# MarioPasc/MU-Diff

Measured on AMD Instinct MI355X. Metric: 256x256 slices/sec (4-step dual-gen reverse), higher is better.
Workload: dtype f32 (convs/attention: fp16 hi+lo split MFMA x3; 3x3 convs that fill the chip: fp16 hi.hi + e4m3 cross terms; fp32 accumulate); 1 GPU; BASELINE config 3 (BraTS-shaped test-split batches of 32; model and slice shapes of config 2): 4-step dual-generator sampling, 256x256, nf=64, ch_mult 1-2-4, 32 slices per GPU per step, batch-sharded over 1 GPU(s), weights replicated; batch=32, hipgraph=True

## Files before the change

### include/mudiff_hip.h

```cpp
#ifndef MUDIFF_HIP_H
#define MUDIFF_HIP_H

#include <stdint.h>

#ifdef __cplusplus
extern "C" {
#endif

#define MUD_OK 0
#define MUD_ERR_ARG 1
#define MUD_ERR_LAUNCH 2
#define MUD_ERR_UNSUPPORTED 3

#define MUD_ACT_NONE 0
#define MUD_ACT_SIGMOID 1
#define MUD_ACT_TANH 2
#define MUD_ACT_SILU 3
#define MUD_ACT_LRELU 4

#define MUD_PRO_NONE 0
#define MUD_PRO_AFFINE 1
#define MUD_PRO_AFFINE_SILU 2
#define MUD_PRO_LRELU 3
#define MUD_PRO_UP2_AFFINE_SILU 4
// ... 56 lines not shown
  int sub2;
  double* stats; int stats_ld;
  int emul_cout;
  const double* gn_sums; int gn_sums_ld;
  int gn_G; float gn_eps; double gn_count;
  const float* gn_gamma; const float* gn_beta;
  int64_t gn_bstride;
  void* splitk_ws; int64_t splitk_ws_bytes;
  unsigned* splitk_counters; int splitk_ncounters;
  const void* skip_w; const float* skip_bias; float* skip_out; int skip_ldo;
  int prec; int w_exp;
  int res_up2; float res_k[4];
  int in_up2; float in_k[4];
  int in_s2d;
} mud_conv_args;

int mud_conv2d_direct(const mud_conv_args* a, void* stream);

int64_t mud_packed_weight_bytes(int ks, int Cin, int Cout);
int mud_pack_weights(const float* src, int64_t s_tap, int64_t s_ci, int64_t s_co, int64_t src_bstride,
                     int ks, int Cin, int Cout, int nbatch, void* dst, void* stream);
int mud_pack_weights_prec(const float* src, int64_t s_tap, int64_t s_ci, int64_t s_co, int64_t src_bstride,
                          int ks, int Cin, int Cout, int nbatch, int prec, int w_exp, void* dst, void* stream);
int64_t mud_packed_weight_bytes_prec(int ks, int Cin, int Cout, int prec);
int mud_conv2d_mfma(const mud_conv_args* a, void* stream);
int mud_conv2d_mfma_prec_supported(const mud_conv_args* a, int prec);
int64_t mud_conv2d_mfma_splitk_bytes(const mud_conv_args* a);
int mud_conv2d_mfma_res_up2_supported(const mud_conv_args* a);
int mud_conv2d_mfma_in_up2_supported(const mud_conv_args* a);
int mud_conv2d_mfma_in_s2d_supported(const mud_conv_args* a);

typedef struct mud_census_args {
  const float* x; int B, H, W, C, ldx;
  const float* pro_scale; const float* pro_shift; int pro_ld; int pro_mode;
} mud_census_args;
typedef struct mud_census_out {
  uint64_t n, n_over, n_under, n_fp16_over, amax_bits;
} mud_census_out;
int mud_e4m3_census(const mud_census_args* a, mud_census_out* out, void* stream);

int mud_upfirdn2d(const float* in, int64_t planes, int H, int W, const float* kernel, int kh, int kw,
                  int up_x, int up_y, int down_x, int down_y, int pad_x0, int pad_x1, int pad_y0, int pad_y1,
                  float* out, void* stream);
int mud_fir_nhwc(const float* x, int B, int H, int W, int C, int ldx, const float* kernel_host, int kh, int kw,
                 int up, int down, int pad0, int pad1,
                 const float* pro_scale, const float* pro_shift, int pro_ld, int pro_mode,
                 float* out_h, int ldh, float* out_x, int ldxo, void* stream);

int mud_minibatch_stddev(const float* x, int B, int64_t hw, int C, int ld, int group, float* out, void* stream);

int mud_attention_supported(int C);
int64_t mud_attention_ws_bytes(int B, int N, int C);
int mud_attention(const float* qkv, int B, int N, int C, int ld, float scale, float* out, int ldo, void* ws, void* stream);

int mud_softmax_rows(float* s, int64_t rows, int n, int ld, void* stream);
int mud_mul(const float* a, int lda, const float* b, int ldb, float* out, int ldo, int64_t npix, int C, void* stream);
int mud_gate_mix(const float* g, int ldg, const float* att, int lda, const float* other, int ldb,
                 float* out, int ldo, int B, int64_t hw, int C, double* stats, int stats_ld, void* stream);

int mud_fourier_embedding(const float* t, const float* W, float* out, int B, int n, void* stream);
int mud_resize_bilinear(const float* in, int64_t planes, int H, int W, int Ho, int Wo, float* out, void* stream);
int mud_affine_clamp(const float* x, int64_t n, float scale, float shift, float lo, float hi, float* out, void* stream);

int64_t mud_value_range_ws_bytes(void);
int mud_value_range(const float* a, int64_t na, const float* b, int64_t nb, float* out, void* ws, void* stream);
int mud_quantize_u8(const float* x, int64_t n, float lo, float range, uint8_t* out, void* stream);
int64_t mud_slice_metrics_ws_bytes(int n, int H, int W);
int mud_slice_metrics_u8(const uint8_t* pred, const uint8_t* gt, int n, int H, int W, int64_t* sse, int64_t* sae, double* ssim_sum,
                         void* ws, int64_t ws_bytes, void* stream);

#define MUD_VM_MAX_REGIONS 8
#define MUD_VM_NQ 8
#define MUD_VM_N 0
#define MUD_VM_SSE 1
#define MUD_VM_SAE 2
#define MUD_VM_N_INT 3
#define MUD_VM_SSIM 4
#define MUD_VM_SS 5
#define MUD_VM_SS2 6
#define MUD_VM_SSE_STD 7
int64_t mud_volume_metrics_ws_bytes(int Z, int X, int Y, int nreg);
int mud_volume_metrics(const float* pred, const float* gt, const uint8_t* region, const float* std, int Z, int X, int Y, int nreg,
                       double* sums, void* ws, int64_t ws_bytes, void* stream);

int64_t mud_lpips_packed_bytes(void);
int mud_lpips_pack(const float* table, void* const* conv_w, void* const* conv_b, void* const* lin_w, void* packed, void* stream);
int64_t mud_lpips_ws_bytes(int n, int H, int W);
int mud_lpips_u8(const uint8_t* pred, const uint8_t* gt, int n, int H, int W, const void* packed, double* out, void* ws,
                 int64_t ws_bytes, void* stream);

int mud_randn_keyed(float* out, int rows, int64_t row_len, const int64_t* keys, uint64_t seed, int step, int kind, void* stream);
int mud_ensemble_stats(const float* samples, int n, int N, int64_t hw, float scale, float shift, float lo, float hi, float* mean,
                       float* std, void* stream);

#define MUD_ENSEMBLE_MAX_QUANTILES 8
#define MUD_ENSEMBLE_QUANTILES_MAX_N 64
int mud_ensemble_quantiles(const float* samples, int n, int N, int64_t hw, float scale, float shift, float lo, float hi, const double* q,
                           int K, float* out, void* stream);

#define MUD_VC_NC 5
#define MUD_VC_NS 2
#define MUD_VC_PARTS 16
#define MUD_VC_N 0
#define MUD_VC_BELOW 1
#define MUD_VC_ABOVE 2
#define MUD_VC_INSIDE 3
// ... 136 lines not shown
```

### mu-diff_amd/csrc/attention.hip

```cpp
#include "mud_common.h"
#include <stdlib.h>

template <int C16>
struct AtGeo {
  static constexpr int C = 16 * C16;
  static constexpr int CT = (C16 + 1) / 2;
  static constexpr int CP = CT * 32;
  static constexpr int KROW = C * 4 + 16;
  static constexpr int VROW = 144;
  static constexpr int KT = 32 * KROW, VT = CP * VROW;
  static constexpr int BUF = KT + VT;
  static constexpr int LDS_BYTES = 2 * BUF;
  static constexpr int KITEMS = 32 * (C / 4), KN = (KITEMS + 255) / 256;
  static constexpr int VITEMS = CP * 8, VN = (VITEMS + 255) / 256;
};

template <int C16>
__global__ __launch_bounds__(256, 1) void k_attention(const float* __restrict__ qkv, int N, int ld, float scale_log2,
                                                       float* __restrict__ out, int ldo, int tiles_per_split, float* __restrict__ part) {
  using G = AtGeo<C16>;
  constexpr int C = G::C, CT = G::CT;
  extern __shared__ __attribute__((aligned(16))) char smem[];
  const int tid = threadIdx.x, lane = tid & 63, wave = tid >> 6, r = lane & 31, hh = lane >> 5;
  const int b = blockIdx.y;
// ... 170 lines not shown
    }

    if (more) stash_v(nxt);
    __syncthreads();
  }

  const float l_tot = l_run + __shfl_xor(l_run, 32, 64);
  if (part) {
    if (qi < N) {
      float* pp = part + (((int64_t)b * gridDim.z + blockIdx.z) * N + qi) * (C + 4);
#pragma unroll
      for (int ct = 0; ct < CT; ++ct)
#pragma unroll
        for (int q4 = 0; q4 < 4; ++q4) {
          const int c0 = ct * 32 + 8 * q4 + 4 * hh;
          if (c0 < C) *(f32x4*)(pp + c0) = f32x4{o[ct][4 * q4], o[ct][4 * q4 + 1], o[ct][4 * q4 + 2], o[ct][4 * q4 + 3]};
        }
      if (hh == 0) { pp[C] = m_run; pp[C + 1] = l_tot; }
    }
    return;
  }
  const float inv = 1.0f / l_tot;
  if (qi < N) {
    float* op = out + ((int64_t)b * N + qi) * ldo;
#pragma unroll
    for (int ct = 0; ct < CT; ++ct)
#pragma unroll
      for (int q4 = 0; q4 < 4; ++q4) {
        const int c0 = ct * 32 + 8 * q4 + 4 * hh;
        if (c0 < C) {
          f32x4 v = {o[ct][4 * q4] * inv, o[ct][4 * q4 + 1] * inv, o[ct][4 * q4 + 2] * inv, o[ct][4 * q4 + 3] * inv};
          *(f32x4*)(op + c0) = v;
        }
      }
  }
}

template <int C16>
struct At2Geo {
  static_assert(C16 % 4 == 0 && C16 >= 8, "pair variant: C in {128, 256}");
  static constexpr int C = 16 * C16;
  static constexpr int H16 = C16 / 2;
  static constexpr int CTH = C16 / 4;
  static constexpr int KROW = C * 4 + 16;
  static constexpr int VROW = 144;
  static constexpr int KT = 32 * KROW, VT = C * VROW;
  static constexpr int V_OFF = 2 * KT, X_OFF = V_OFF + VT;
  static constexpr int LDS_BYTES = X_OFF + 8 * 4096;
  static constexpr int KN = (32 * (C / 4)) / 512;
  static constexpr int VN = (C * 8) / 512;
  static_assert(KN * 512 == 32 * (C / 4) && VN * 512 == C * 8, "staging split");
};

template <int C16>
__global__ __launch_bounds__(512, 2) void k_attention_pair(const float* __restrict__ qkv, int N, int ld, float scale_log2,
                                                            float* __restrict__ out, int ldo, int tiles_per_split, float* __restrict__ part) {
  using G = At2Geo<C16>;
  constexpr int C = G::C, H16 = G::H16, CTH = G::CTH;
  extern __shared__ __attribute__((aligned(16))) char smem[];
  const int tid = threadIdx.x, lane = tid & 63, wave = tid >> 6, r = lane & 31, hh = lane >> 5;
  const int pair = wave & 3, half = wave >> 2;
  const int b = blockIdx.y;
  const int qi = blockIdx.x * 128 + pair * 32 + r;
  const float* base = qkv + (int64_t)b * N * ld;
  const int kt0 = blockIdx.z * tiles_per_split;
  const int ntiles = min((N + 31) / 32, kt0 + tiles_per_split);

  mud_h16x8 qh[H16], ql[H16];
#pragma unroll
  for (int s = 0; s < H16; ++s) {
    f32x4 v0 = {0.f, 0.f, 0.f, 0.f}, v1 = {0.f, 0.f, 0.f, 0.f};
    if (qi < N) {
      const float* qp = base + (int64_t)qi * ld + 16 * (half * H16 + s) + 8 * hh;
      v0 = *(const f32x4*)qp;
      v1 = *(const f32x4*)(qp + 4);
    }
#pragma unroll
    for (int e = 0; e < 4; ++e) {
      mud_h16 h0, h1, l0, l1;
      mud_split1(v0[e], h0, l0);
      mud_split1(v1[e], h1, l1);
      qh[s][e] = h0; qh[s][4 + e] = h1;
      ql[s][e] = l0; ql[s][4 + e] = l1;
    }
  }

  const __amdgpu_buffer_rsrc_t rsrc = __builtin_amdgcn_make_buffer_rsrc((void*)base, 0, (int)((int64_t)N * ld * 4 < 0x7fffffffLL ? (int64_t)N * ld * 4 : 0x7fffffffLL), 0x00020000);
  constexpr int KJ = 512 / (C / 4);
  constexpr int VG = 512 / C;
  const unsigned kvoff = (unsigned)(((tid / (C / 4)) * ld + C + 4 * (tid % (C / 4))) * 4);
  const unsigned vvoff = (unsigned)((2 * C + (tid % C)) * 4 + (4 * (tid / C)) * ld * 4);
  f32x4 kraw[G::KN];
  float vraw[G::VN][4];
  auto fetch_k = [&](int kt) {
#pragma unroll
    for (int i = 0; i < G::KN; ++i)
      kraw[i] = __builtin_bit_cast(f32x4, __builtin_amdgcn_raw_buffer_load_b128(rsrc, kvoff, (kt * 32 + KJ * i) * ld * 4, 0));
  };
  auto fetch_v = [&](int kt) {
#pragma unroll
    for (int i = 0; i < G::VN; ++i)
#pragma unroll
      for (int u = 0; u < 4; ++u)
        vraw[i][u] = __builtin_bit_cast(float, __builtin_amdgcn_raw_buffer_load_b32(rsrc, vvoff, (kt * 32 + 4 * VG * i + u) * ld * 4, 0));
  };
  auto stash_k = [&](char* buf) {
#pragma unroll
    for (int i = 0; i < G::KN; ++i) {
      const int item = tid + 512 * i, j = item / (C / 4), c4 = item % (C / 4);
      mud_h16x4 hi, lo;
      mud_split4(kraw[i], hi, lo);
      *(mud_h16x4*)(buf + j * G::KROW + c4 * 8) = hi;
      *(mud_h16x4*)(buf + j * G::KROW + C * 2 + c4 * 8) = lo;
    }
  };
  auto stash_v = [&]() {
#pragma unroll
    for (int i = 0; i < G::VN; ++i) {
      const int item = tid + 512 * i, c = item % C, g = item / C;
      const int jj = (4 * g) & 15, s = (4 * g) >> 4, h = (jj >> 2) & 1, blk = (jj >> 3) & 1;
      mud_h16x4 hi, lo;
#pragma unroll
      for (int u = 0; u < 4; ++u) {
        mud_h16 th, tl;
        mud_split1(vraw[i][u], th, tl);
        hi[u] = th;
        lo[u] = tl;
      }
      char* p = smem + G::V_OFF + c * G::VROW + s * 32 + h * 16 + blk * 8;
      *(mud_h16x4*)p = hi;
      *(mud_h16x4*)(p + 64) = lo;
    }
  };

  f32x16 o[CTH];
#pragma unroll
  for (int ct = 0; ct < CTH; ++ct)
#pragma unroll
    for (int i = 0; i < 16; ++i) o[ct][i] = 0.f;
  float m_run = -INFINITY, l_run = 0.f;
  f32x4* const xmine = (f32x4*)(smem + G::X_OFF + wave * 4096) + lane;
  const f32x4* const xpeer = (const f32x4*)(smem + G::X_OFF + (wave ^ 4) * 4096) + lane;

  fetch_k(kt0);
  stash_k(smem);
  fetch_v(kt0);
  stash_v();
  __syncthreads();

  for (int kt = kt0; kt < ntiles; ++kt) {
    const char* cur = smem + ((kt - kt0) & 1) * G::KT;
    char* nxt = smem + ((kt - kt0 + 1) & 1) * G::KT;
    const bool more = kt + 1 < ntiles;
    if (more) fetch_k(kt + 1);

    f32x16 st;
#pragma unroll
    for (int i = 0; i < 16; ++i) st[i] = 0.f;
#pragma unroll
    for (int s = 0; s < H16; ++s) {
      const char* kp = cur + r * G::KROW + (16 * (half * H16 + s) + 8 * hh) * 2;
      const mud_h16x8 kh = *(const mud_h16x8*)kp;
      const mud_h16x8 kl = *(const mud_h16x8*)(kp + C * 2);
      st = mud_mfma16(kl, qh[s], st);
      st = mud_mfma16(kh, ql[s], st);
      st = mud_mfma16(kh, qh[s], st);
    }
#pragma unroll
    for (int q4 = 0; q4 < 4; ++q4) xmine[q4 * 64] = f32x4{st[4 * q4], st[4 * q4 + 1], st[4 * q4 + 2], st[4 * q4 + 3]};
    if (more) {
      stash_k(nxt);
      fetch_v(kt + 1);
    }
    __syncthreads();
#pragma unroll
    for (int q4 = 0; q4 < 4; ++q4) {
      const f32x4 p = xpeer[q4 * 64];
      if (half == 0) { st[4 * q4] += p[0]; st[4 * q4 + 1] += p[1]; st[4 * q4 + 2] += p[2]; st[4 * q4 + 3] += p[3]; }
      else { st[4 * q4] = p[0] + st[4 * q4]; st[4 * q4 + 1] = p[1] + st[4 * q4 + 1]; st[4 * q4 + 2] = p[2] + st[4 * q4 + 2]; st[4 * q4 + 3] = p[3] + st[4 * q4 + 3]; }
    }

    float mt = -INFINITY;
#pragma unroll
    for (int i = 0; i < 16; ++i) {
      const int key = kt * 32 + (i & 3) + 8 * (i >> 2) + 4 * hh;
      st[i] = key < N ? st[i] * scale_log2 : -INFINITY;
      mt = fmaxf(mt, st[i]);
    }
    mt = fmaxf(mt, __shfl_xor(mt, 32, 64));
    const float m_new = fmaxf(m_run, mt);
    const float alpha = __builtin_amdgcn_exp2f(m_run - m_new);
    float psum = 0.f;
#pragma unroll
    for (int i = 0; i < 16; ++i) {
      st[i] = __builtin_amdgcn_exp2f(st[i] - m_new);
      psum += st[i];
    }
    l_run = l_run * alpha + psum;
    m_run = m_new;
    if (!__all(alpha == 1.0f)) {
#pragma unroll
      for (int ct = 0; ct < CTH; ++ct)
#pragma unroll
        for (int i = 0; i < 16; ++i) o[ct][i] *= alpha;
    }
    mud_h16x8 ph[2], pl[2];
#pragma unroll
    for (int s2 = 0; s2 < 2; ++s2)
#pragma unroll
      for (int e = 0; e < 8; ++e) {
        const float p = st[8 * s2 + e];
        const mud_h16 t = (mud_h16)p;
        ph[s2][e] = t;
        pl[s2][e] = (mud_h16)(p - (float)t);
      }

#pragma unroll
    for (int ct = 0; ct < CTH; ++ct) {
#pragma unroll
      for (int s2 = 0; s2 < 2; ++s2) {
        const char* vp = smem + G::V_OFF + ((half * CTH + ct) * 32 + r) * G::VROW + s2 * 32 + hh * 16;
        const mud_h16x8 vh = *(const mud_h16x8*)vp;
        const mud_h16x8 vl = *(const mud_h16x8*)(vp + 64);
        o[ct] = mud_mfma16(vl, ph[s2], o[ct]);
        o[ct] = mud_mfma16(vh, pl[s2], o[ct]);
        o[ct] = mud_mfma16(vh, ph[s2], o[ct]);
      }
    }
    __syncthreads();
    if (more) stash_v();
  }

  const float l_tot = l_run + __shfl_xor(l_run, 32, 64);
  if (part) {
    if (qi < N) {
      float* pp = part + (((int64_t)b * gridDim.z + blockIdx.z) * N + qi) * (C + 4);
#pragma unroll
      for (int ct = 0; ct < CTH; ++ct)
#pragma unroll
        for (int q4 = 0; q4 < 4; ++q4) {
          const int c0 = (half * CTH + ct) * 32 + 8 * q4 + 4 * hh;
          *(f32x4*)(pp + c0) = f32x4{o[ct][4 * q4], o[ct][4 * q4 + 1], o[ct][4 * q4 + 2], o[ct][4 * q4 + 3]};
        }
      if (hh == 0 && half == 0) { pp[C] = m_run; pp[C + 1] = l_tot; }
    }
    return;
  }
  const float inv = 1.0f / l_tot;
  if (qi < N) {
    float* op = out + ((int64_t)b * N + qi) * ldo;
#pragma unroll
    for (int ct = 0; ct < CTH; ++ct)
#pragma unroll
      for (int q4 = 0; q4 < 4; ++q4) {
        const int c0 = (half * CTH + ct) * 32 + 8 * q4 + 4 * hh;
        *(f32x4*)(op + c0) = f32x4{o[ct][4 * q4] * inv, o[ct][4 * q4 + 1] * inv, o[ct][4 * q4 + 2] * inv, o[ct][4 * q4 + 3] * inv};
      }
  }
}

__global__ __launch_bounds__(256) void k_attention_combine(const float* __restrict__ part, int N, int C, int nsplit, float* __restrict__ out, int ldo) {
  const int C4 = C / 4;
  const unsigned t = blockIdx.x * 256u + threadIdx.x;
  if (t >= (unsigned)(N * C4)) return;
  const int q = (int)(t / (unsigned)C4), c = (int)(t - (unsigned)q * (unsigned)C4) * 4, b = blockIdx.y;
  const int64_t row = C + 4;
  const float* p0 = part + ((int64_t)b * nsplit * N + q) * row;
  float m = -INFINITY;
  for (int s = 0; s < nsplit; ++s) m = fmaxf(m, p0[(int64_t)s * N * row + C]);
  f32x4 acc = {0.f, 0.f, 0.f, 0.f};
  float l = 0.f;
  for (int s = 0; s < nsplit; ++s) {
    const float* ps = p0 + (int64_t)s * N * row;
    const float w = __builtin_amdgcn_exp2f(ps[C] - m);
    acc += w * *(const f32x4*)(ps + c);
    l += w * ps[C + 1];
  }
  *(f32x4*)(out + ((int64_t)b * N + q) * ldo + c) = acc * (1.0f / l);
}

static int at_splits(int B, int N) {
  const int64_t wgs = (int64_t)B * mud_cdiv(N, 128);
  const int ntiles = (int)mud_cdiv(N, 32);
  if (ntiles < 8) return 1;
  int best = 1;
  double best_cost = (double)mud_cdiv(wgs, 256);
  for (int ns = 2; ns <= 16 && ns <= ntiles / 4; ++ns) {
    const double cost = (double)mud_cdiv(wgs * ns, 256) / ns + 0.01 * ns;
    if (cost < best_cost - 1e-9) best_cost = cost, best = ns;
  }
  const int tps = (int)mud_cdiv(ntiles, best);
  return (int)mud_cdiv(ntiles, tps);
}

template <int C16>
static int at_launch_pair(const float* qkv, int B, int N, int ld, float scale, float* out, int ldo, float* ws, hipStream_t s) {
  using G = At2Geo<C16>;
  static mud_attr_once attr_once;
  if (attr_once.need()) {
    hipError_t e = hipFuncSetAttribute((const void*)k_attention_pair<C16>, hipFuncAttributeMaxDynamicSharedMemorySize, G::LDS_BYTES);
    if (e != hipSuccess) {
      mud_set_error("mud_attention: cannot reserve %d B of LDS: %s", G::LDS_BYTES, hipGetErrorString(e));
      return MUD_ERR_LAUNCH;
    }
    attr_once.ok();
  }
  const int ntiles = (int)mud_cdiv(N, 32);
  const int ns = ws ? at_splits(B, N) : 1;
  const int tps = (int)mud_cdiv(ntiles, ns);
  hipLaunchKernelGGL((k_attention_pair<C16>), dim3((unsigned)mud_cdiv(N, 128), B, ns), dim3(512), G::LDS_BYTES, s, qkv, N, ld,
                     scale * 1.44269504088896340736f, out, ldo, tps, ns > 1 ? ws : (float*)nullptr);
  MUD_CHECK_LAUNCH("mud_attention(pair)");
  if (ns > 1) {
    hipLaunchKernelGGL(k_attention_combine, dim3((unsigned)mud_cdiv((int64_t)N * (G::C / 4), 256), B), dim3(256), 0, s, ws, N, G::C, ns, out, ldo);
    MUD_CHECK_LAUNCH("mud_attention(combine)");
  }
  return MUD_OK;
}

template <int C16>
static int at_launch(const float* qkv, int B, int N, int ld, float scale, float* out, int ldo, float* ws, hipStream_t s) {
  using G = AtGeo<C16>;
  static mud_attr_once attr_once;
  if (attr_once.need()) {
    hipError_t e = hipFuncSetAttribute((const void*)k_attention<C16>, hipFuncAttributeMaxDynamicSharedMemorySize, G::LDS_BYTES);
    if (e != hipSuccess) {
      mud_set_error("mud_attention: cannot reserve %d B of LDS: %s", G::LDS_BYTES, hipGetErrorString(e));
      return MUD_ERR_LAUNCH;
    }
    attr_once.ok();
  }
  const int ntiles = (int)mud_cdiv(N, 32);
  const int ns = ws ? at_splits(B, N) : 1;
  const int tps = (int)mud_cdiv(ntiles, ns);
  hipLaunchKernelGGL((k_attention<C16>), dim3((unsigned)mud_cdiv(N, 128), B, ns), dim3(256), G::LDS_BYTES, s, qkv, N, ld,
                     scale * 1.44269504088896340736f, out, ldo, tps, ns > 1 ? ws : (float*)nullptr);
  MUD_CHECK_LAUNCH("mud_attention");
  if (ns > 1) {
    hipLaunchKernelGGL(k_attention_combine, dim3((unsigned)mud_cdiv((int64_t)N * (G::C / 4), 256), B), dim3(256), 0, s, ws, N, G::C, ns, out, ldo);
    MUD_CHECK_LAUNCH("mud_attention(combine)");
  }
  return MUD_OK;
}

extern "C" int64_t mud_attention_ws_bytes(int B, int N, int C) {
  if (B <= 0 || N <= 0 || C <= 0) return 0;
  const int ns = at_splits(B, N);
  return ns > 1 ? (int64_t)B * ns * N * (C + 4) * 4 : 0;
}

extern "C" int mud_attention_supported(int C) { return C == 16 || C == 32 || C == 64 || C == 128 || C == 256; }

extern "C" int mud_attention(const float* qkv, int B, int N, int C, int ld, float scale, float* out, int ldo, void* ws, void* stream) {
  MUD_REQUIRE(qkv && out, "mud_attention: null pointer");
  MUD_REQUIRE(B >= 0 && B <= 65535 && N > 0 && ld >= 3 * C && ldo >= C, "mud_attention: bad sizes");
  MUD_REQUIRE(mud_attention_supported(C), "mud_attention: head dim %d not in {16,32,64,128,256}", C);
  MUD_REQUIRE(ld % 4 == 0 && ldo % 4 == 0 && mud_aligned16(qkv) && mud_aligned16(out) && mud_aligned16(ws), "mud_attention: needs ld %% 4 == 0 and 16-byte aligned buffers");
  if (B == 0) return MUD_OK;
  hipStream_t s = (hipStream_t)stream;
  static const bool at_pair = !(getenv("MUD_ATT_SINGLE") && atoi(getenv("MUD_ATT_SINGLE")));
  switch (C) {
    case 16: return at_launch<1>(qkv, B, N, ld, scale, out, ldo, (float*)ws, s);
    case 32: return at_launch<2>(qkv, B, N, ld, scale, out, ldo, (float*)ws, s);
    case 64: return at_launch<4>(qkv, B, N, ld, scale, out, ldo, (float*)ws, s);
    case 128: return at_pair ? at_launch_pair<8>(qkv, B, N, ld, scale, out, ldo, (float*)ws, s) : at_launch<8>(qkv, B, N, ld, scale, out, ldo, (float*)ws, s);
    default: return at_pair ? at_launch_pair<16>(qkv, B, N, ld, scale, out, ldo, (float*)ws, s) : at_launch<16>(qkv, B, N, ld, scale, out, ldo, (float*)ws, s);
  }
}
```

### mu-diff_amd/mudiff_hip/__init__.py

```python
from __future__ import annotations

import ctypes as C
import os

import torch

_HERE = os.path.dirname(os.path.abspath(__file__))
_SHIPPED = os.path.join(_HERE, 'libmudiff_hip.so')
_LIB_PATH = os.environ.get('MUDIFF_HIP_LIB', _SHIPPED)
_lib = None
PREC_16X3, PREC_FP8X, PREC_16X1 = 0, 1, 2

ACT_NONE, ACT_SIGMOID, ACT_TANH, ACT_SILU, ACT_LRELU = 0, 1, 2, 3, 4
PRO_NONE, PRO_AFFINE, PRO_AFFINE_SILU, PRO_LRELU = 0, 1, 2, 3


class MudiffHipError(RuntimeError):
    pass


class ConvArgs(C.Structure):
    _fields_ = [
        ('x', C.c_void_p), ('B', C.c_int), ('H', C.c_int), ('W', C.c_int), ('Cin', C.c_int), ('ldx', C.c_int),
        ('w', C.c_void_p), ('w_bstride', C.c_int64),
# ... 43 lines not shown
class CensusOut(C.Structure):
    _fields_ = [('n', C.c_uint64), ('n_over', C.c_uint64), ('n_under', C.c_uint64), ('n_fp16_over', C.c_uint64), ('amax_bits', C.c_uint64)]


VI_MAX_RANKS, VI_WINDOW = 4, 16
NIFTI_U1, NIFTI_I2, NIFTI_I4, NIFTI_F4, NIFTI_U2 = 2, 4, 8, 16, 512


class VolumeCensusRecord(C.Structure):
    _fields_ = [('n', C.c_uint64), ('n_nonfinite', C.c_uint64), ('min', C.c_float), ('max', C.c_float),
                ('count', C.c_int32 * VI_MAX_RANKS), ('first_rank', C.c_int64 * VI_MAX_RANKS),
                ('window', (C.c_float * VI_WINDOW) * VI_MAX_RANKS)]


class BandTables(C.Structure):
    _fields_ = [('m', C.c_int), ('n', C.c_int), ('bw', C.c_int), ('nnz', C.c_int),
                ('start', C.c_void_p), ('member', C.c_void_p), ('w', C.c_void_p),
                ('tstart', C.c_void_p), ('tmember', C.c_void_p), ('tw', C.c_void_p), ('lc', C.c_void_p)]


_P, _I, _L, _F, _D = C.c_void_p, C.c_int, C.c_int64, C.c_float, C.c_double
_SIGNATURES = {
    'mud_version': (C.c_int, []),
    'mud_last_error': (C.c_char_p, []),
    'mud_build_flags': (C.c_char_p, []),
    'mud_posterior_sample': (_I, [_P, _P, _P, _P, _P, _P, _P, _P, _I, _P, _I, _L, _P]),
    'mud_q_sample': (_I, [_P, _P, _P, _I, _P, _P, _I, _P, _I, _L, _P]),
    'mud_timestep_embedding': (_I, [_P, _P, _I, _I, _F, _P]),
    'mud_pixel_norm': (_I, [_P, _P, _I, _I, _P]),
    'mud_dense': (_I, [_P, _I, _P, _P, _P, _I, _I, _I, _I, _I, _I, _P]),
    'mud_mlp_chain': (_I, [C.POINTER(MlpArgs), _P]),
    'mud_mlp_chains': (_I, [C.POINTER(MlpArgs), _I, _P]),
    'mud_gn_ws_bytes': (_L, [_I, _L, _I, _I]),
    'mud_gn_scale_shift': (_I, [_P, _I, _L, _I, _I, _I, _F, _P, _P, _L, _P, _P, _I, _P, _P, _P]),
    'mud_gn_scale_shift_from_sums': (_I, [_P, _I, _I, _I, _I, C.c_double, _F, _P, _P, _L, _P, _P, _I, _P]),
    'mud_channel_mean': (_I, [_P, _I, _L, _I, _I, _P, _I, _P, _P]),
    'mud_conv2d_direct': (_I, [C.POINTER(ConvArgs), _P]),
    'mud_packed_weight_bytes': (_L, [_I, _I, _I]),
    'mud_pack_weights': (_I, [_P, _L, _L, _L, _L, _I, _I, _I, _I, _P, _P]),
    'mud_pack_weights_prec': (_I, [_P, _L, _L, _L, _L, _I, _I, _I, _I, _I, _I, _P, _P]),
    'mud_packed_weight_bytes_prec': (_L, [_I, _I, _I, _I]),
    'mud_conv2d_mfma': (_I, [C.POINTER(ConvArgs), _P]),
    'mud_conv2d_mfma_prec_supported': (_I, [C.POINTER(ConvArgs), _I]),
    'mud_conv2d_mfma_splitk_bytes': (_L, [C.POINTER(ConvArgs)]),
    'mud_conv2d_mfma_res_up2_supported': (_I, [C.POINTER(ConvArgs)]),
    'mud_conv2d_mfma_in_up2_supported': (_I, [C.POINTER(ConvArgs)]),
    'mud_conv2d_mfma_in_s2d_supported': (_I, [C.POINTER(ConvArgs)]),
    'mud_upfirdn2d': (_I, [_P, _L, _I, _I, _P, _I, _I, _I, _I, _I, _I, _I, _I, _I, _I, _P, _P]),
    'mud_fir_nhwc': (_I, [_P, _I, _I, _I, _I, _I, C.POINTER(C.c_float), _I, _I, _I, _I, _I, _I, _P, _P, _I, _I, _P, _I, _P, _I, _P]),
    'mud_minibatch_stddev': (_I, [_P, _I, _L, _I, _I, _I, _P, _P]),
    'mud_attention_supported': (_I, [_I]),
    'mud_attention_ws_bytes': (_L, [_I, _I, _I]),
    'mud_attention': (_I, [_P, _I, _I, _I, _I, _F, _P, _I, _P, _P]),
    'mud_softmax_rows': (_I, [_P, _L, _I, _I, _P]),
    'mud_mul': (_I, [_P, _I, _P, _I, _P, _I, _L, _I, _P]),
    'mud_gate_mix': (_I, [_P, _I, _P, _I, _P, _I, _P, _I, _I, _L, _I, _P, _I, _P]),
    'mud_fourier_embedding': (_I, [_P, _P, _P, _I, _I, _P]),
    'mud_resize_bilinear': (_I, [_P, _L, _I, _I, _I, _I, _P, _P]),
    'mud_affine_clamp': (_I, [_P, _L, _F, _F, _F, _F, _P, _P]),
    'mud_e4m3_census': (_I, [C.POINTER(CensusArgs), _P, _P]),
    'mud_value_range_ws_bytes': (_L, []),
    'mud_value_range': (_I, [_P, _L, _P, _L, _P, _P, _P]),
    'mud_quantize_u8': (_I, [_P, _L, _F, _F, _P, _P]),
    'mud_slice_metrics_ws_bytes': (_L, [_I, _I, _I]),
    'mud_slice_metrics_u8': (_I, [_P, _P, _I, _I, _I, _P, _P, _P, _P, _L, _P]),
    'mud_volume_metrics_ws_bytes': (_L, [_I, _I, _I, _I]),
    'mud_volume_metrics': (_I, [_P, _P, _P, _P, _I, _I, _I, _I, _P, _P, _L, _P]),
    'mud_lpips_packed_bytes': (_L, []),
    'mud_lpips_pack': (_I, [_P, _P, _P, _P, _P, _P]),
    'mud_lpips_ws_bytes': (_L, [_I, _I, _I]),
    'mud_lpips_u8': (_I, [_P, _P, _I, _I, _I, _P, _P, _P, _L, _P]),
    'mud_randn_keyed': (_I, [_P, _I, _L, _P, C.c_uint64, _I, _I, _P]),
    'mud_ensemble_stats': (_I, [_P, _I, _I, _L, _F, _F, _F, _F, _P, _P, _P]),
    'mud_ensemble_quantiles': (_I, [_P, _I, _I, _L, _F, _F, _F, _F, C.POINTER(C.c_double), _I, _P, _P]),
    'mud_volume_interval_coverage': (_I, [_P, _P, _P, _P, _I, _I, _I, _I, _I, _I, _P, _P, _P, _L, _P]),
    'mud_randn_keyed_coupled': (_I, [_P, _I, _L, _P, C.c_uint64, _I, _I, C.POINTER(C.c_double), _I, _P]),
    'mud_known_constrain': (_I, [_P, _P, _P, _P, _P, C.c_uint64, _I, _I, _P, _I, _P, _P, _I, _I, _P, _I, _L, _P]),
    'mud_known_coverage': (_I, [C.POINTER(C.c_double), _I, _I, _I, _I, _I, _I, _P, _P]),
    'mud_fft2_c2c': (_I, [_P, _P, _I, _I, _I, _P]),
    'mud_fft2_r2c': (_I, [_P, _P, _I, _I, _I, _P]),
    'mud_kspace_constrain': (_I, [_P, _P, _P, _I, _P, _P, C.c_uint64, _I, _I, _P, _I, _P, _P, _I, _I, _P, _P, _I, _I, _P]),
    'mud_slab_constrain': (_I, [_P, _P, _P, _P, _P, _I, _I, _P, _P, C.c_uint64, _I, _I, _P, _I, _P, _P, _I, _I, _P, _I, _L, _P]),
    'mud_slab_average': (_I, [_P, _P, _P, _I, _I, _P, _I, _L, _P]),
    'mud_slab_kspace_constrain': (_I, [_P, _P, _P, _I, _P, _P, _P, _I, _I, _P, _P, C.c_uint64, _I, _I, _P, _I, _P, _P, _I, _I, _P, _P, _I, _I,
                                        _P]),
    'mud_band_constrain': (_I, [_P, _P, C.POINTER(BandTables), _P, _P, C.c_uint64, _I, _I, _P, _I, _P, _P, _I, _I, _P, _P, _I, _L, _P]),
    'mud_band_measure': (_I, [_P, C.POINTER(BandTables), _P, _I, _L, _P]),
    'mud_volume_through_plane': (_I, [_P, _P, _I, _I, _I, _I, _I, _P, _P, _L, _P]),
    'mud_volume_census_ws_bytes': (_L, []),
    'mud_volume_census': (_I, [_P, _I, _I, _I, _I, _F, _F, C.POINTER(C.c_double), _I, _P, _P, _L, _P]),
    'mud_volume_slab_normalise': (_I, [_P, _I, _I, _I, _I, _F, _F, _F, _F, _I, _I, _I, _P, _P]),
    'mud_volume_slab_zscore': (_I, [_P, _I, _I, _I, _I, _F, _F, _F, _F, _I, _I, _P, _P]),
    'mud_volume_assemble': (_I, [_P, _P, _I, _I, _I, _I, _I, _P, _P, _P]),
    'mud_volume_regrid': (_I, [_P, _I, _I, _I, _I, _F, _F, C.POINTER(C.c_double), _I, _I, _I, _I, _P, _P]),
    'mud_volume_bspline_coeffs': (_I, [_P, _I, _I, _I, _I, _F, _F, _P, _P, _P]),
    'mud_volume_regrid_cubic': (_I, [_P, _I, _I, _I, _P, _I, _F, _F, C.POINTER(C.c_double), _D, _D, _I, _I, _I, _P, _P]),
    'mud_volume_joint_hist': (_I, [_P, _I, _I, _I, _I, _F, _F, _P, _I, _I, _I, _I, _F, _F, C.POINTER(C.c_double), _I, _D, _D, _D, _D, _I, _P, _P]),
    'mud_volume_mirror_moments': (_I, [_P, _I, _I, _I, _I, _F, _F, _P, _I, _I, _D, _D, _I, _P, _P]),
    'mud_volume_bias_log': (_I, [_P, _I, _I, _I, _I, _F, _F, _I, _P, _P]),
    'mud_volume_bias_corrected': (_I, [_P, _P, _P, _P, _I, _I, _I, _I, _I, _P, _P]),
    'mud_volume_bias_hist': (_I, [_P, _L, _D, _D, _I, _P, _P]),
    'mud_volume_bias_fit': (_I, [_P, _P, _I, _D, _D, _I, _I, _I, _I, _I, _I, _P, _P]),
    'mud_volume_bias_apply': (_I, [_P, _I, _I, _I, _I, _F, _F, _P, _I, _I, _P, _P]),
    'mud_volume_denoise_residual': (_I, [_P, _I, _I, _I, _I, _F, _F, _P, _P]),
    'mud_volume_denoise_select_hist': (_I, [_P, _L, C.c_uint32, _I, _P, _P]),
    'mud_volume_denoise_nlm': (_I, [_P, _I, _I, _I, _I, _F, _F, _I, _I, _D, _D, _I, _P, _P, _P]),
# ... 67 lines not shown
```

### mu-diff_amd/mudiff_hip/ops.py

```python
from __future__ import annotations

import collections
import ctypes as C
import math
import os

import numpy as np
import torch

from . import (ACT_LRELU, ACT_NONE, ACT_SIGMOID, ACT_SILU, ACT_TANH, PREC_16X1, PREC_16X3, PREC_FP8X, PRO_AFFINE, PRO_AFFINE_SILU, PRO_LRELU,
               PRO_NONE, ConvArgs, MudiffHipError, check, load, ptr, require_gpu)


DETERMINISTIC = os.environ.get('MUD_DETERMINISTIC', '0') == '1'


class StatsArena:

    def __init__(self, device, chunk_doubles=1 << 18):
        self.device, self.chunk = device, chunk_doubles
        self.buf, self.used = None, 0

    def take(self, B, C):
        if DETERMINISTIC:
# ... 603 lines not shown
    else:
        sc, sh, mode = resolve_pro(pro)
        a.pro_mode = mode
        if mode != PRO_NONE:
            assert sc.shape == (x.B, x.C) and sc.stride(1) == 1 and sh.stride() == sc.stride(), (tuple(sc.shape), sc.stride(), sh.stride())
            a.pro_scale, a.pro_shift, a.pro_ld = ptr(sc), ptr(sh), sc.stride(0)
    _launch('e4m3_census', x.device, load().mud_e4m3_census, C.byref(a), ptr(out), STREAM, nbytes=4.0 * x.npix * x.C)
    return out


def upfirdn2d_planes(x, kernel, up, down, pad):
    require_gpu(x, kernel)
    N, Cc, H, W = x.shape
    xin = _f32(x.float().contiguous())
    k = _f32(kernel.float().contiguous())
    kh, kw = k.shape
    (ux, uy), (dx, dy), (px0, px1, py0, py1) = up, down, pad
    Ho = (H * uy + py0 + py1 - kh) // dy + 1
    Wo = (W * ux + px0 + px1 - kw) // dx + 1
    out = torch.empty(N, Cc, Ho, Wo, device=x.device, dtype=torch.float32)
    _launch('upfirdn2d', x.device, load().mud_upfirdn2d, ptr(xin), N * Cc, H, W, ptr(k), kh, kw, ux, uy, dx, dy, px0, px1, py0, py1, ptr(out), STREAM)
    return out.to(x.dtype)


def fir_nhwc(x: View, kernel2d, up, down, pad, pro=None, want_h=True, want_x=False):
    import numpy as np
    k = np.ascontiguousarray(kernel2d, dtype=np.float32)
    kh, kw = k.shape
    Ho = (x.H * up + pad[0] + pad[1] - kh) // down + 1
    Wo = (x.W * up + pad[0] + pad[1] - kw) // down + 1
    oh = View.empty(x.B, Ho, Wo, x.C, x.device) if want_h else None
    ox = View.empty(x.B, Ho, Wo, x.C, x.device) if want_x else None
    sc = sh = None
    ld = mode = 0
    if pro is not None:
        sc, sh, mode = resolve_pro(pro)
        ld = sc.stride(0)
    _launch('fir_nhwc', x.device, load().mud_fir_nhwc, x.ptr, x.B, x.H, x.W, x.C, x.ld, k.ctypes.data_as(C.POINTER(C.c_float)), kh, kw, up, down,
            pad[0], pad[1], ptr(sc), ptr(sh), ld, mode, oh.ptr if oh else None, oh.ld if oh else 0, ox.ptr if ox else None,
            ox.ld if ox else 0, STREAM, nbytes=4.0 * x.C * (x.npix + x.B * Ho * Wo * (int(want_h) + int(want_x))))
    return oh, ox


def minibatch_stddev(x: View, group):
    out = torch.empty(x.B, device=x.device, dtype=torch.float32)
    _launch('minibatch_stddev', x.device, load().mud_minibatch_stddev, x.ptr, x.B, x.H * x.W, x.C, x.ld, group, ptr(out), STREAM)
    return out


def attention_supported(C_):
    return bool(load().mud_attention_supported(C_))


def attention(qkv: View, C_, scale):
    assert qkv.C == 3 * C_
    n = qkv.H * qkv.W
    out = View.empty(qkv.B, qkv.H, qkv.W, C_, qkv.device)
    nws = load().mud_attention_ws_bytes(qkv.B, n, C_)
    ws = torch.empty(nws // 4, device=qkv.device, dtype=torch.float32) if nws else None
    _launch('attention', qkv.device, load().mud_attention, qkv.ptr, qkv.B, n, C_, qkv.ld, float(scale), out.ptr, out.ld, ptr(ws) if nws else None,
            STREAM, flops=4.0 * qkv.B * n * n * C_)
    return out


def softmax_rows_(s, n):
    rows = s.numel() // n
    _launch('softmax_rows', s.device, load().mud_softmax_rows, ptr(s), rows, n, n, STREAM)
    return s


def mul(a: View, b: View, out: View = None):
    out = View.empty(a.B, a.H, a.W, a.C, a.device) if out is None else out
    _launch('mul', a.device, load().mud_mul, a.ptr, a.ld, b.ptr, b.ld, out.ptr, out.ld, a.npix, a.C, STREAM)
    return out


def gate_mix(g: View, att: View, other: View, out: View):
    _launch('gate_mix', g.device, load().mud_gate_mix, g.ptr, g.ld, att.ptr, att.ld, other.ptr, other.ld, out.ptr, out.ld, g.B, g.H * g.W, g.C,
            out.stats_ptr, out.stats.shape[1] if out.stats is not None else 0, STREAM)
    return out


def resize_bilinear(x, size):
    require_gpu(x)
    H, W = x.shape[-2:]
    Ho, Wo = int(size[0]), int(size[1])
    xin = _f32(x.float().contiguous())
    out = torch.empty(*x.shape[:-2], Ho, Wo, device=x.device, dtype=torch.float32)
    _launch('resize_bilinear', x.device, load().mud_resize_bilinear, ptr(xin), xin.numel() // (H * W), H, W, Ho, Wo, ptr(out), STREAM)
    return out


def affine_clamp(x, scale, shift, lo, hi):
    require_gpu(x)
    xin = _f32(x.float().contiguous())
    out = torch.empty_like(xin)
    _launch('affine_clamp', x.device, load().mud_affine_clamp, ptr(xin), xin.numel(), float(scale), float(shift), float(lo), float(hi), ptr(out), STREAM)
    return out


def value_range(a, b=None):
    require_gpu(a, b)
    ain = _f32(a.contiguous())
    bin_ = None if b is None else _f32(b.contiguous())
    out = torch.empty(2, device=a.device, dtype=torch.float32)
    ws = torch.empty(load().mud_value_range_ws_bytes(), device=a.device, dtype=torch.uint8)
    _launch('value_range', a.device, load().mud_value_range, ptr(ain), ain.numel(), ptr(bin_), 0 if bin_ is None else bin_.numel(),
            ptr(out), ptr(ws), STREAM)
    return out


def quantize_u8(x, gmin, gmax):
    require_gpu(x)
    gmin, gmax = float(gmin), float(gmax)
# ... 944 lines not shown
```

Baseline: 109.3 slices/s.

## Pre-split K/V into fp16 hi/lo tile images before pair attention

Adds a prepass kernel that converts each 32-key tile of K and V into fp16 hi/lo halves, laid out exactly as the pair attention kernel's LDS tiles. The attention kernel can then stream those images with 128-bit loads and copy them straight to LDS. This removes the repeated strided fp32 loads and per-block hi/lo splitting that every query block used to redo. It also skips the key-bound masking on all but a ragged last tile. The cost is an extra kernel launch, a workspace allocation and an extra write/read of the images, so the path is enabled only when there are at least 24 query blocks.

```diff
diff --git a/include/mudiff_hip.h b/include/mudiff_hip.h
--- a/include/mudiff_hip.h
+++ b/include/mudiff_hip.h
@@ -132,6 +132,9 @@
 int mud_attention_supported(int C);
 int64_t mud_attention_ws_bytes(int B, int N, int C);
 int mud_attention(const float* qkv, int B, int N, int C, int ld, float scale, float* out, int ldo, void* ws, void* stream);
+int64_t mud_attention_images_bytes(int B, int N, int C);
+int mud_attention_split_kv(const float* qkv, int B, int N, int C, int ld, void* images, void* stream);
+int mud_attention_v2(const float* qkv, int B, int N, int C, int ld, float scale, float* out, int ldo, void* ws, const void* images, void* stream);
 
 int mud_softmax_rows(float* s, int64_t rows, int n, int ld, void* stream);
 int mud_mul(const float* a, int lda, const float* b, int ldb, float* out, int ldo, int64_t npix, int C, void* stream);
diff --git a/mu-diff_amd/csrc/attention.hip b/mu-diff_amd/csrc/attention.hip
--- a/mu-diff_amd/csrc/attention.hip
+++ b/mu-diff_amd/csrc/attention.hip
@@ -246,9 +246,10 @@
   static_assert(KN * 512 == 32 * (C / 4) && VN * 512 == C * 8, "staging split");
 };
 
-template <int C16>
+template <int C16, bool PRE>
 __global__ __launch_bounds__(512, 2) void k_attention_pair(const float* __restrict__ qkv, int N, int ld, float scale_log2,
-                                                            float* __restrict__ out, int ldo, int tiles_per_split, float* __restrict__ part) {
+                                                            float* __restrict__ out, int ldo, int tiles_per_split, float* __restrict__ part,
+                                                            const char* __restrict__ images) {
   using G = At2Geo<C16>;
   constexpr int C = G::C, H16 = G::H16, CTH = G::CTH;
   extern __shared__ __attribute__((aligned(16))) char smem[];
@@ -284,23 +285,40 @@
   constexpr int VG = 512 / C;
   const unsigned kvoff = (unsigned)(((tid / (C / 4)) * ld + C + 4 * (tid % (C / 4))) * 4);
   const unsigned vvoff = (unsigned)((2 * C + (tid % C)) * 4 + (4 * (tid / C)) * ld * 4);
+  constexpr int TILE = 128 * C;
+  static_assert(G::KN * 512 * 16 == TILE && G::VN * 512 * 16 == TILE, "image tile = KN (VN) 16-byte pieces per thread");
+  const int tiles_all = (N + 31) / 32;
+  const __amdgpu_buffer_rsrc_t irsrc = __builtin_amdgcn_make_buffer_rsrc((void*)(PRE ? images + (int64_t)b * 2 * tiles_all * TILE : nullptr), 0,
+                                                                         PRE ? 2 * tiles_all * TILE : 0, 0x00020000);
   f32x4 kraw[G::KN];
   float vraw[G::VN][4];
+  f32x4 vimg[G::VN];
   auto fetch_k = [&](int kt) {
 #pragma unroll
-    for (int i = 0; i < G::KN; ++i)
-      kraw[i] = __builtin_bit_cast(f32x4, __builtin_amdgcn_raw_buffer_load_b128(rsrc, kvoff, (kt * 32 + KJ * i) * ld * 4, 0));
+    for (int i = 0; i < G::KN; ++i) {
+      if constexpr (PRE) kraw[i] = __builtin_bit_cast(f32x4, __builtin_amdgcn_raw_buffer_load_b128(irsrc, tid * 16, kt * TILE + i * 8192, 0));
+      else kraw[i] = __builtin_bit_cast(f32x4, __builtin_amdgcn_raw_buffer_load_b128(rsrc, kvoff, (kt * 32 + KJ * i) * ld * 4, 0));
+    }
   };
   auto fetch_v = [&](int kt) {
 #pragma unroll
-    for (int i = 0; i < G::VN; ++i)
-#pragma unroll
-      for (int u = 0; u < 4; ++u)
-        vraw[i][u] = __builtin_bit_cast(float, __builtin_amdgcn_raw_buffer_load_b32(rsrc, vvoff, (kt * 32 + 4 * VG * i + u) * ld * 4, 0));
+    for (int i = 0; i < G::VN; ++i) {
+      if constexpr (PRE) vimg[i] = __builtin_bit_cast(f32x4, __builtin_amdgcn_raw_buffer_load_b128(irsrc, tid * 16, (tiles_all + kt) * TILE + i * 8192, 0));
+      else {
+#pragma unroll
+        for (int u = 0; u < 4; ++u)
+          vraw[i][u] = __builtin_bit_cast(float, __builtin_amdgcn_raw_buffer_load_b32(rsrc, vvoff, (kt * 32 + 4 * VG * i + u) * ld * 4, 0));
+      }
+    }
   };
   auto stash_k = [&](char* buf) {
 #pragma unroll
     for (int i = 0; i < G::KN; ++i) {
+      if constexpr (PRE) {
+        const int item = tid + 512 * i, j = item / (C / 4), c = item % (C / 4);
+        *(f32x4*)(buf + j * G::KROW + c * 16) = kraw[i];
+        continue;
+      }
       const int item = tid + 512 * i, j = item / (C / 4), c4 = item % (C / 4);
       mud_h16x4 hi, lo;
       mud_split4(kraw[i], hi, lo);
@@ -311,6 +329,11 @@
   auto stash_v = [&]() {
 #pragma unroll
     for (int i = 0; i < G::VN; ++i) {
+      if constexpr (PRE) {
+        const int item = tid + 512 * i;
+        *(f32x4*)(smem + G::V_OFF + (item >> 3) * G::VROW + (item & 7) * 16) = vimg[i];
+        continue;
+      }
       const int item = tid + 512 * i, c = item % C, g = item / C;
       const int jj = (4 * g) & 15, s = (4 * g) >> 4, h = (jj >> 2) & 1, blk = (jj >> 3) & 1;
       mud_h16x4 hi, lo;
@@ -375,12 +398,18 @@
     }
 
     float mt = -INFINITY;
-#pragma unroll
-    for (int i = 0; i < 16; ++i) {
-      const int key = kt * 32 + (i & 3) + 8 * (i >> 2) + 4 * hh;
-      st[i] = key < N ? st[i] * scale_log2 : -INFINITY;
-      mt = fmaxf(mt, st[i]);
-    }
+    if ((N & 31) != 0 && kt == tiles_all - 1) {
+#pragma unroll
+      for (int i = 0; i < 16; ++i) {
+        const int key = kt * 32 + (i & 3) + 8 * (i >> 2) + 4 * hh;
+        st[i] = key < N ? st[i] * scale_log2 : -INFINITY;
+      }
+    } else {
+#pragma unroll
+      for (int i = 0; i < 16; ++i) st[i] *= scale_log2;
+    }
+#pragma unroll
+    for (int i = 0; i < 16; ++i) mt = fmaxf(mt, st[i]);
     mt = fmaxf(mt, __shfl_xor(mt, 32, 64));
     const float m_new = fmaxf(m_run, mt);
     const float alpha = __builtin_amdgcn_exp2f(m_run - m_new);
@@ -450,6 +479,48 @@
         const int c0 = (half * CTH + ct) * 32 + 8 * q4 + 4 * hh;
         *(f32x4*)(op + c0) = f32x4{o[ct][4 * q4] * inv, o[ct][4 * q4 + 1] * inv, o[ct][4 * q4 + 2] * inv, o[ct][4 * q4 + 3] * inv};
       }
+  }
+}
+
+template <int C>
+__global__ __launch_bounds__(256) void k_attention_split_kv(const float* __restrict__ qkv, int N, int ld, char* __restrict__ images) {
+  constexpr int TILE = 128 * C, PASSES = (4 * C) / 256;
+  const int tid = threadIdx.x, t = blockIdx.x, T = gridDim.x, b = blockIdx.y;
+  const float* base = qkv + (int64_t)b * N * ld;
+  char* kimg = images + ((int64_t)b * 2 * T + t) * TILE;
+  char* vimg = images + ((int64_t)b * 2 * T + T + t) * TILE;
+#pragma unroll
+  for (int i = 0; i < PASSES; ++i) {
+    const int item = tid + 256 * i, j = item / (C / 8), c8 = item % (C / 8), key = t * 32 + j;
+    f32x4 v0 = {0.f, 0.f, 0.f, 0.f}, v1 = {0.f, 0.f, 0.f, 0.f};
+    if (key < N) {
+      const float* p = base + (int64_t)key * ld + C + 8 * c8;
+      v0 = *(const f32x4*)p;
+      v1 = *(const f32x4*)(p + 4);
+    }
+    mud_h16x4 h0, l0, h1, l1;
+    mud_split4(v0, h0, l0);
+    mud_split4(v1, h1, l1);
+    char* o = kimg + j * (4 * C) + c8 * 16;
+    *(mud_h16x8*)o = __builtin_shufflevector(h0, h1, 0, 1, 2, 3, 4, 5, 6, 7);
+    *(mud_h16x8*)(o + 2 * C) = __builtin_shufflevector(l0, l1, 0, 1, 2, 3, 4, 5, 6, 7);
+  }
+#pragma unroll
+  for (int i = 0; i < PASSES; ++i) {
+    const int item = tid + 256 * i, q = item & 3, c = item >> 2, s = q >> 1, h = q & 1;
+    mud_h16x8 hi, lo;
+#pragma unroll
+    for (int e = 0; e < 8; ++e) {
+      const int key = t * 32 + 16 * s + 8 * (e >> 2) + 4 * h + (e & 3);
+      const float v = key < N ? base[(int64_t)key * ld + 2 * C + c] : 0.f;
+      mud_h16 th, tl;
+      mud_split1(v, th, tl);
+      hi[e] = th;
+      lo[e] = tl;
+    }
+    char* o = vimg + c * 128 + q * 16;
+    *(mud_h16x8*)o = hi;
+    *(mud_h16x8*)(o + 64) = lo;
   }
 }
 
@@ -487,12 +558,12 @@
   return (int)mud_cdiv(ntiles, tps);
 }
 
-template <int C16>
-static int at_launch_pair(const float* qkv, int B, int N, int ld, float scale, float* out, int ldo, float* ws, hipStream_t s) {
+template <int C16, bool PRE>
+static int at_launch_pair(const float* qkv, int B, int N, int ld, float scale, float* out, int ldo, float* ws, const char* images, hipStream_t s) {
   using G = At2Geo<C16>;
   static mud_attr_once attr_once;
   if (attr_once.need()) {
-    hipError_t e = hipFuncSetAttribute((const void*)k_attention_pair<C16>, hipFuncAttributeMaxDynamicSharedMemorySize, G::LDS_BYTES);
+    hipError_t e = hipFuncSetAttribute((const void*)k_attention_pair<C16, PRE>, hipFuncAttributeMaxDynamicSharedMemorySize, G::LDS_BYTES);
     if (e != hipSuccess) {
       mud_set_error("mud_attention: cannot reserve %d B of LDS: %s", G::LDS_BYTES, hipGetErrorString(e));
       return MUD_ERR_LAUNCH;
@@ -502,8 +573,8 @@
   const int ntiles = (int)mud_cdiv(N, 32);
   const int ns = ws ? at_splits(B, N) : 1;
   const int tps = (int)mud_cdiv(ntiles, ns);
-  hipLaunchKernelGGL((k_attention_pair<C16>), dim3((unsigned)mud_cdiv(N, 128), B, ns), dim3(512), G::LDS_BYTES, s, qkv, N, ld,
-                     scale * 1.44269504088896340736f, out, ldo, tps, ns > 1 ? ws : (float*)nullptr);
+  hipLaunchKernelGGL((k_attention_pair<C16, PRE>), dim3((unsigned)mud_cdiv(N, 128), B, ns), dim3(512), G::LDS_BYTES, s, qkv, N, ld,
+                     scale * 1.44269504088896340736f, out, ldo, tps, ns > 1 ? ws : (float*)nullptr, images);
   MUD_CHECK_LAUNCH("mud_attention(pair)");
   if (ns > 1) {
     hipLaunchKernelGGL(k_attention_combine, dim3((unsigned)mud_cdiv((int64_t)N * (G::C / 4), 256), B), dim3(256), 0, s, ws, N, G::C, ns, out, ldo);
@@ -545,19 +616,52 @@
 
 extern "C" int mud_attention_supported(int C) { return C == 16 || C == 32 || C == 64 || C == 128 || C == 256; }
 
-extern "C" int mud_attention(const float* qkv, int B, int N, int C, int ld, float scale, float* out, int ldo, void* ws, void* stream) {
+static bool at_images_fit(int N, int C) { return mud_cdiv(N, 32) * 256 * C < 0x7fffffffLL; }
+
+extern "C" int64_t mud_attention_images_bytes(int B, int N, int C) {
+  if (B <= 0 || N <= 0 || C <= 0) return 0;
+  return (int64_t)B * mud_cdiv(N, 32) * 256 * C;
+}
+
+extern "C" int mud_attention_split_kv(const float* qkv, int B, int N, int C, int ld, void* images, void* stream) {
+  MUD_REQUIRE(qkv && images, "mud_attention_split_kv: null pointer");
+  MUD_REQUIRE(B >= 0 && B <= 65535 && N > 0 && ld >= 3 * C, "mud_attention_split_kv: bad sizes");
+  MUD_REQUIRE(C == 128 || C == 256, "mud_attention_split_kv: head dim %d not in {128,256} (the pair kernel's)", C);
+  MUD_REQUIRE(at_images_fit(N, C), "mud_attention_split_kv: the images of one sample must stay below 2 GiB (N = %d, C = %d)", N, C);
+  MUD_REQUIRE(ld % 4 == 0 && mud_aligned16(qkv) && mud_aligned16(images), "mud_attention_split_kv: needs ld %% 4 == 0 and 16-byte aligned buffers");
+  if (B == 0) return MUD_OK;
+  const dim3 grid((unsigned)mud_cdiv(N, 32), B);
+  if (C == 128) hipLaunchKernelGGL(k_attention_split_kv<128>, grid, dim3(256), 0, (hipStream_t)stream, qkv, N, ld, (char*)images);
+  else hipLaunchKernelGGL(k_attention_split_kv<256>, grid, dim3(256), 0, (hipStream_t)stream, qkv, N, ld, (char*)images);
+  MUD_CHECK_LAUNCH("mud_attention_split_kv");
+  return MUD_OK;
+}
+
+extern "C" int mud_attention_v2(const float* qkv, int B, int N, int C, int ld, float scale, float* out, int ldo, void* ws, const void* images, void* stream) {
   MUD_REQUIRE(qkv && out, "mud_attention: null pointer");
   MUD_REQUIRE(B >= 0 && B <= 65535 && N > 0 && ld >= 3 * C && ldo >= C, "mud_attention: bad sizes");
   MUD_REQUIRE(mud_attention_supported(C), "mud_attention: head dim %d not in {16,32,64,128,256}", C);
   MUD_REQUIRE(ld % 4 == 0 && ldo % 4 == 0 && mud_aligned16(qkv) && mud_aligned16(out) && mud_aligned16(ws), "mud_attention: needs ld %% 4 == 0 and 16-byte aligned buffers");
+  static const bool at_pair = !(getenv("MUD_ATT_SINGLE") && atoi(getenv("MUD_ATT_SINGLE")));
+  const bool pair = at_pair && (C == 128 || C == 256);
+  MUD_REQUIRE(!images || ((C == 128 || C == 256) && at_images_fit(N, C) && mud_aligned16(images)),
+              "mud_attention: split images are read by the pair kernel only (C in {128,256}), 16-byte aligned, below 2 GiB per sample");
   if (B == 0) return MUD_OK;
   hipStream_t s = (hipStream_t)stream;
-  static const bool at_pair = !(getenv("MUD_ATT_SINGLE") && atoi(getenv("MUD_ATT_SINGLE")));
+  const char* img = pair ? (const char*)images : nullptr;
   switch (C) {
     case 16: return at_launch<1>(qkv, B, N, ld, scale, out, ldo, (float*)ws, s);
     case 32: return at_launch<2>(qkv, B, N, ld, scale, out, ldo, (float*)ws, s);
     case 64: return at_launch<4>(qkv, B, N, ld, scale, out, ldo, (float*)ws, s);
-    case 128: return at_pair ? at_launch_pair<8>(qkv, B, N, ld, scale, out, ldo, (float*)ws, s) : at_launch<8>(qkv, B, N, ld, scale, out, ldo, (float*)ws, s);
-    default: return at_pair ? at_launch_pair<16>(qkv, B, N, ld, scale, out, ldo, (float*)ws, s) : at_launch<16>(qkv, B, N, ld, scale, out, ldo, (float*)ws, s);
-  }
-}
+    case 128:
+      if (!pair) return at_launch<8>(qkv, B, N, ld, scale, out, ldo, (float*)ws, s);
+      return img ? at_launch_pair<8, true>(qkv, B, N, ld, scale, out, ldo, (float*)ws, img, s) : at_launch_pair<8, false>(qkv, B, N, ld, scale, out, ldo, (float*)ws, img, s);
+    default:
+      if (!pair) return at_launch<16>(qkv, B, N, ld, scale, out, ldo, (float*)ws, s);
+      return img ? at_launch_pair<16, true>(qkv, B, N, ld, scale, out, ldo, (float*)ws, img, s) : at_launch_pair<16, false>(qkv, B, N, ld, scale, out, ldo, (float*)ws, img, s);
+  }
+}
+
+extern "C" int mud_attention(const float* qkv, int B, int N, int C, int ld, float scale, float* out, int ldo, void* ws, void* stream) {
+  return mud_attention_v2(qkv, B, N, C, ld, scale, out, ldo, ws, nullptr, stream);
+}
diff --git a/mu-diff_amd/mudiff_hip/__init__.py b/mu-diff_amd/mudiff_hip/__init__.py
--- a/mu-diff_amd/mudiff_hip/__init__.py
+++ b/mu-diff_amd/mudiff_hip/__init__.py
@@ -119,6 +119,9 @@
     'mud_attention_supported': (_I, [_I]),
     'mud_attention_ws_bytes': (_L, [_I, _I, _I]),
     'mud_attention': (_I, [_P, _I, _I, _I, _I, _F, _P, _I, _P, _P]),
+    'mud_attention_images_bytes': (_L, [_I, _I, _I]),
+    'mud_attention_split_kv': (_I, [_P, _I, _I, _I, _I, _P, _P]),
+    'mud_attention_v2': (_I, [_P, _I, _I, _I, _I, _F, _P, _I, _P, _P, _P]),
     'mud_softmax_rows': (_I, [_P, _L, _I, _I, _P]),
     'mud_mul': (_I, [_P, _I, _P, _I, _P, _I, _L, _I, _P]),
     'mud_gate_mix': (_I, [_P, _I, _P, _I, _P, _I, _P, _I, _I, _L, _I, _P, _I, _P]),
diff --git a/mu-diff_amd/mudiff_hip/ops.py b/mu-diff_amd/mudiff_hip/ops.py
--- a/mu-diff_amd/mudiff_hip/ops.py
+++ b/mu-diff_amd/mudiff_hip/ops.py
@@ -679,14 +679,24 @@
     return bool(load().mud_attention_supported(C_))
 
 
+ATT_PRESPLIT = os.environ.get('MUD_ATT_PRESPLIT', '1') != '0'
+ATT_PRESPLIT_MIN_QBLOCKS = 24
+
+
 def attention(qkv: View, C_, scale):
     assert qkv.C == 3 * C_
     n = qkv.H * qkv.W
+    lib = load()
     out = View.empty(qkv.B, qkv.H, qkv.W, C_, qkv.device)
-    nws = load().mud_attention_ws_bytes(qkv.B, n, C_)
+    nws = lib.mud_attention_ws_bytes(qkv.B, n, C_)
     ws = torch.empty(nws // 4, device=qkv.device, dtype=torch.float32) if nws else None
-    _launch('attention', qkv.device, load().mud_attention, qkv.ptr, qkv.B, n, C_, qkv.ld, float(scale), out.ptr, out.ld, ptr(ws) if nws else None,
-            STREAM, flops=4.0 * qkv.B * n * n * C_)
+    images = None
+    if ATT_PRESPLIT and C_ in (128, 256) and qkv.B > 0 and -(-n // 128) >= ATT_PRESPLIT_MIN_QBLOCKS:
+        images = torch.empty(lib.mud_attention_images_bytes(qkv.B, n, C_), device=qkv.device, dtype=torch.uint8)
+        _launch('attention_split_kv', qkv.device, lib.mud_attention_split_kv, qkv.ptr, qkv.B, n, C_, qkv.ld, ptr(images), STREAM,
+                nbytes=16.0 * qkv.B * n * C_)
+    _launch('attention', qkv.device, lib.mud_attention_v2, qkv.ptr, qkv.B, n, C_, qkv.ld, float(scale), out.ptr, out.ld, ptr(ws) if nws else None,
+            ptr(images) if images is not None else None, STREAM, flops=4.0 * qkv.B * n * n * C_)
     return out
 
 
```

Result: no change. 109.7 slices/s (median of 6 runs) (+0.3%).
